# BadgerTechnologies/navigation

Hardware: AMD Instinct MI355X
Metric: scored trajectories/sec (whole node) + costmap inflation cells/sec, 400x400 map (higher is better)
Workload: dtype f64

## Files before the change

### navigation_amd/csrc/planner_score.h

```cpp
#pragma once
#include "planner_common.h"

namespace navgpu {

__host__ __device__ inline size_t score_bits_bytes(int win) {
  return (((size_t)4 * win * ((win + 31) >> 5) * 4) + 15) & ~(size_t)15;
}
__host__ __device__ inline size_t score_scratch_bytes(int win) { return score_bits_bytes(win); }
__device__ __forceinline__ int divSmall(int n, int d) {
  int q = (int)((float)n * __builtin_amdgcn_rcpf((float)d));
  int r = n - q * d;
  if (r < 0) {
    --q;
    r += d;
  }
  if (r >= d) ++q;
  return q;
}

struct WorldToMapFast {
  const Geom& g;
  const double& inv_res;
  __device__ __forceinline__ bool operator()(double wx, double wy, uint32_t& mx, uint32_t& my) const {
    const double dx = wx - g.ox, dy = wy - g.oy;
    const double qx = dx * inv_res, qy = dy * inv_res;
    double fx = floor(qx), fy = floor(qy);
    const double rx = qx - fx, ry = qy - fy;
    if (__builtin_expect(fmin(rx, ry) < 1.0e-7 || fmax(rx, ry) > 1.0 - 1.0e-7, 0)) {
      fx = !(dx >= 0.0) ? -1.0 : (qx >= 1.0e6 ? 1.0e6 : (double)(int)(dx / g.res));
      fy = !(dy >= 0.0) ? -1.0 : (qy >= 1.0e6 ? 1.0e6 : (double)(int)(dy / g.res));
    }
    int ix, iy;
    asm("v_cvt_i32_f64 %0, %1" : "=v"(ix) : "v"(fx));
    asm("v_cvt_i32_f64 %0, %1" : "=v"(iy) : "v"(fy));
    mx = (uint32_t)ix;
    my = (uint32_t)iy;
    return mx < g.nx && my < g.ny;
  }
};

__device__ __forceinline__ void addCritic(double& total, bool en, double value, double scale) {
  if (!en) return;
  double cost = value;
  if (cost != 0) cost *= scale;
  total += cost;
}

constexpr uint32_t kScoreAuxBytes = 64;
__host__ __device__ inline uint32_t score_prep_reject_bytes(const PlannerDev& pl) { return (pl.max_axis * pl.max_axis + 255u) & ~255u; }
__host__ __device__ inline uint32_t score_prep_reject_offset(const PlannerDev& pl) { return pl.prep_stride - score_prep_reject_bytes(pl); }
template <size_t kAllowAbove = 48 * 1024, typename... P, typename... A>
void launchScore(void (*kernel)(P...), dim3 grid, int threads, size_t lds, hipStream_t s, A... args) {
  if (lds > kAllowAbove) hipFuncSetAttribute((const void*)kernel, hipFuncAttributeMaxDynamicSharedMemorySize, (int)lds);
  hipLaunchKernelGGL(kernel, grid, dim3(threads), lds, s, args...);
}
size_t score_table_row_bytes(const PlannerDev& pl);
size_t score_table_lds_bytes(const PlannerDev& pl);
bool score_sweep_applies(const PlannerDev& pl);
uint32_t launch_score_sweep(const PlannerDev& pl, uint32_t first, uint32_t count, hipStream_t s);

}
```

### navigation_amd/csrc/planner_score.hip

```cpp
#include "planner_score.h"

namespace navgpu {

#ifdef NAVGPU_PREP_TIMING
__device__ unsigned long long g_prep_stats[16];
#define PREP_STAMP(i) prep_t[i] = wall_clock64()
#else
#define PREP_STAMP(i)
#endif

struct ScoreRobot {
  uint32_t inst;
  Geom g;
  navgpu_robot_state st;
  const uint8_t* master;
  const uint32_t *dpath, *dgoal, *dfront;
  const int32_t* cnt;
  uint32_t nfp;
  int win, wx0, wy0;
  int win_bytes, nw;
};
__device__ __forceinline__ ScoreRobot scoreRobot(const PlannerDev& pl, uint32_t inst) {
  ScoreRobot r;
  r.inst = inst;
// ... 200 lines not shown
  for (uint32_t i = threadIdx.x; i < n16; i += blockDim.x) img[i] = lds[i];
}

__device__ __forceinline__ void storeSweepScalars(const PlannerDev& pl, const ScoreRobot& r, const float (*s_axis)[kMaxAxis], int* s_cnt,
                                                  const uint8_t* s_dyn) {
  const uint32_t tid = threadIdx.x;
  const navgpu_dwa_config& c = pl.cfg;
  const Geom& g = r.g;
  const int32_t* cnt = r.cnt;
  const uint32_t inst = r.inst;
  const int win = r.win, wx0 = r.wx0, wy0 = r.wy0, nw = r.nw;
  const uint32_t* s_fb = reinterpret_cast<const uint32_t*>(s_dyn + r.win_bytes);
  uint8_t* rej = pl.prep + (size_t)inst * pl.prep_stride + score_prep_reject_offset(pl);
  int32_t* aux = reinterpret_cast<int32_t*>(rej - kScoreAuxBytes);
  const int c0 = win / 2;
  const uint32_t w_c0 = (uint32_t)(c0 * nw + (c0 >> 5));
  const int start_fail = ((s_fb[4 * w_c0 + 2] >> (c0 & 31)) & 1u) ? 4 : (((s_fb[4 * w_c0 + 3] >> (c0 & 31)) & 1u) ? 5 : 0);
  if (tid == 0) s_cnt[0] = (win / 2) * (win / 2);
  __syncthreads();
  {
    int dmin = win * win;
    for (int it = tid; it < win * nw; it += blockDim.x) {
      const int y = it / nw, j = it - y * nw;
      uint32_t m = (c.sum_scores ? s_fb[4 * it] : s_fb[4 * it + 1]) | (start_fail == 4 ? 0u : s_fb[4 * it + 2]) | (start_fail != 0 ? 0u : s_fb[4 * it + 3]);
      const int dy = y > c0 ? y - c0 : c0 - y;
      const int p = c0 - 32 * j;
      const uint32_t right = p <= 0 ? m : (p >= 32 ? 0u : m & (0xFFFFFFFFu << p)), left = m & ~right;
      if (right) dmin = min(dmin, (32 * j + __ffs(right) - 1 - c0) * (32 * j + __ffs(right) - 1 - c0) + dy * dy);
      if (left) dmin = min(dmin, (c0 - (32 * j + 31 - __clz(left))) * (c0 - (32 * j + 31 - __clz(left))) + dy * dy);
    }
    atomicMin(&s_cnt[0], dmin);
  }
  __syncthreads();
  if (tid == 0) {
    const double inv_res = pl.inv_res, fpd = c.forward_point_distance;
    const bool en_fwd = pl.scale_goal != 0 || (pl.align_on[inst] && pl.scale_path != 0);
    const uint32_t fwd_margin = (uint32_t)fmin(ceil(fabs(fpd) * inv_res) + 1.0, 1.0e6);
    const bool fwd_screen = !en_fwd || (2u * fwd_margin < g.nx && 2u * fwd_margin < g.ny);
    const uint32_t fwd_lo = en_fwd ? fwd_margin : 0u, fwd_nx = g.nx - 2u * fwd_lo, fwd_ny = g.ny - 2u * fwd_lo;
    const bool need_margin = !((uint32_t)wx0 - fwd_lo < fwd_nx && (uint32_t)(wx0 + win - 1) - fwd_lo < fwd_nx && (uint32_t)wy0 - fwd_lo < fwd_ny &&
                               (uint32_t)(wy0 + win - 1) - fwd_lo < fwd_ny);
    aux[0] = wx0;
    aux[1] = wy0;
    aux[2] = (int32_t)fwd_lo;
    aux[3] = (int32_t)fwd_nx;
    aux[4] = (int32_t)fwd_ny;
    aux[5] = need_margin ? 1 : 0;
    aux[6] = fwd_screen ? 1 : 0;
    aux[7] = (int)floor(sqrt((double)s_cnt[0]));
    aux[8] = start_fail;
  }
  const int nyv = max(cnt[1], 1), nxyv = cnt[0] * cnt[1];
  for (int i = tid; i < nxyv; i += blockDim.x) {
    const int ix = i / nyv, iy = i - ix * nyv;
    const double vmag = hyp2((double)s_axis[0][ix], (double)s_axis[1][iy]);
    const double eps = 1e-4;
    rej[i] = (uint8_t)(((c.min_trans_vel >= 0 && vmag + eps < c.min_trans_vel) ? 1 : 0) | ((c.max_trans_vel >= 0 && vmag - eps > c.max_trans_vel) ? 2 : 0));
  }
}

struct ScoreInputs {
  static constexpr int kAxisChunks = (3 * kMaxAxis + kScoreThreads - 1) / kScoreThreads;
  double fp;
  float axis[kAxisChunks];
};
__device__ __forceinline__ ScoreInputs loadInputs(const PlannerDev& pl, const ScoreRobot& r) {
  const uint32_t tid = threadIdx.x;
  ScoreInputs in;
  in.fp = pl.fp_spec[(size_t)r.inst * kMaxFootprint * 2 + (tid < 2 * r.nfp ? tid : 0)];
#pragma unroll
  for (int u = 0; u < ScoreInputs::kAxisChunks; ++u) {
    const uint32_t i = min(tid + (uint32_t)u * kScoreThreads, 3u * kMaxAxis - 1), a = i / kMaxAxis, k = i - a * kMaxAxis;
    in.axis[u] = pl.axis_samples[((size_t)r.inst * 3 + a) * pl.max_axis + min(k, pl.max_axis - 1)];
    if (k >= pl.max_axis) in.axis[u] = 0.f;
  }
  return in;
}
__device__ __forceinline__ void loadImage(const PlannerDev& pl, const ScoreRobot& r, const ScoreInputs& in, double* s_fp, float (*s_axis)[kMaxAxis],
                                          uint8_t* s_dyn) {
  const uint32_t tid = threadIdx.x;
  const uint4* img = reinterpret_cast<const uint4*>(pl.prep + (size_t)r.inst * pl.prep_stride);
  uint4* lds = reinterpret_cast<uint4*>(s_dyn);
  const uint32_t n16 = pl.prep_bytes >> 4;
  for (uint32_t i = tid; i < n16; i += blockDim.x) lds[i] = img[i];
  if (tid < 2 * r.nfp) s_fp[tid] = in.fp;
#pragma unroll
  for (int u = 0; u < ScoreInputs::kAxisChunks; ++u) {
    const uint32_t i = tid + (uint32_t)u * kScoreThreads;
    if (i < 3u * kMaxAxis) s_axis[i / kMaxAxis][i % kMaxAxis] = in.axis[u];
  }
// ... 599 lines not shown
```

### navigation_amd/csrc/planner_score_sweep.hip

```cpp
#include "planner_score.h"

namespace navgpu {

constexpr int kSweepThreads = NAVGPU_SCORE_TAB_THREADS;
constexpr int kSweepWaves = 6;
#ifndef NAVGPU_SWEEP_BLOCK_STEPS
#define NAVGPU_SWEEP_BLOCK_STEPS 4
#endif
#ifndef NAVGPU_SWEEP_QUEUE
#define NAVGPU_SWEEP_QUEUE 768
#endif
constexpr int kSweepBlockSteps = NAVGPU_SWEEP_BLOCK_STEPS;
constexpr int kSweepQueue = NAVGPU_SWEEP_QUEUE;
constexpr uint32_t kWalkFailed = 0x80000000u;
#ifdef NAVGPU_SWEEP_COUNTS
__device__ unsigned long long g_sweep_counts[16];
#define SW_COUNT(slot_, n_)                                                                    \
  do {                                                                                           \
    const unsigned long long swc_ = (unsigned long long)(n_);                                    \
    if ((threadIdx.x & 63u) == 0) atomicAdd(&g_sweep_counts[slot_], swc_);                       \
  } while (0)
#else
#define SW_COUNT(slot_, n_)
#endif
#ifdef NAVGPU_SWEEP_TIMING
__device__ unsigned long long g_sweep_stats[16];
#define SW_STAMP(v) const unsigned long long v = __builtin_amdgcn_s_memtime()
#define SW_ACC(i, x) sw_t[i] += (x)
#else
#define SW_STAMP(v)
#define SW_ACC(i, x)
#endif

template <int CHUNK, bool TRIGF>
__global__ __launch_bounds__(kSweepThreads, kSweepWaves) void k_score_sweep(PlannerDev pl, uint32_t first) {
  constexpr int THREADS = kSweepThreads;
  extern __shared__ __align__(16) uint8_t s_dyn[];
  uint8_t* s_win = s_dyn;
  __shared__ double s_rc[THREADS / 64];
  __shared__ int s_ri[THREADS / 64];
  __shared__ int s_cnt[2];
  __shared__ float s_qx[kSweepQueue], s_qy[kSweepQueue];
  __shared__ uint32_t s_qt[kSweepQueue];
  __shared__ uint32_t s_obs[THREADS];
  __shared__ uint32_t s_qn[2];
  __shared__ uint32_t s_more[3];

  const uint32_t inst = first + blockIdx.z;
  const uint32_t tid = threadIdx.x;
#ifdef NAVGPU_SWEEP_TIMING
  unsigned long long sw_t[10] = {0, 0, 0, 0, 0, 0, 0, 0, 0, 0};
#endif
  SW_STAMP(sw0);
  __builtin_amdgcn_s_setprio(3);
  const navgpu_dwa_config& c = pl.cfg;
  const Geom g = geomOf(pl, inst);
  const navgpu_robot_state st = pl.state[inst];
  const uint8_t* master = pl.master + (size_t)inst * pl.cells_padded;
  const uint32_t* dpath = pl.path + (size_t)inst * pl.cells;
  const uint32_t* dgoal = pl.goal + (size_t)inst * pl.cells;
  const uint32_t* dfront = pl.goal_front + (size_t)inst * pl.cells;
  const int32_t* cnt = pl.axis_count + 4 * inst;
  const int n_samples = cnt[3];
  const uint32_t nfp = pl.fp_n[inst];
  const int win = (int)pl.win;

  if (tid == 0) s_cnt[0] = s_cnt[1] = 0;
  if (tid < 2) s_qn[tid] = 0;
  if (tid < 3) s_more[tid] = 0;
  s_obs[tid] = 0;
  const uint8_t* rej_bytes = pl.prep + (size_t)inst * pl.prep_stride + score_prep_reject_offset(pl);
  const int32_t* aux = reinterpret_cast<const int32_t*>(rej_bytes - kScoreAuxBytes);
  const int wx0 = aux[0], wy0 = aux[1];
  const uint32_t fwd_lo = (uint32_t)aux[2], fwd_nx = (uint32_t)aux[3], fwd_ny = (uint32_t)aux[4];
  const bool need_margin = aux[5] != 0, fwd_screen = aux[6] != 0;
  const int free_cells = aux[7];
  const int start_fail = aux[8];
  const uint32_t osc = pl.osc_flags[inst];
  const int32_t align_on = pl.align_on[inst];
  const int win_bytes = (win * win + 15) & ~15;
  const int nw = (win + 31) >> 5;
  const bool walk_swap = pl.cfg.allow_unknown != 0;
  const uint32_t walk_fail = walk_swap ? 255u : 254u;
  const int K = (int)pl.tab_steps;
  const int tnfp = (int)pl.tab_nfp;
  const int lrows = (int)pl.tab_rows;
  double* s_trig = reinterpret_cast<double*>(s_dyn + win_bytes + score_bits_bytes(win));
  double* s_rot = s_trig + (size_t)lrows * K * 4;
  const int nxy = max(cnt[0] * cnt[1], 1);
  const uint32_t part_slot = blockIdx.y * gridDim.x + blockIdx.x;
  const int t_row_base = (int)blockIdx.y * (int)pl.tab_rows;
  const int t_rows = min(max(cnt[2] - t_row_base, 0), (int)pl.tab_rows);
  const int t_li0 = (int)blockIdx.x * THREADS;
  if (t_li0 >= t_rows * nxy) {
    if (tid == 0) {
      pl.part_cost[(size_t)inst * pl.score_blocks + part_slot] = 1.0e300;
      pl.part_index[(size_t)inst * pl.score_blocks + part_slot] = 0x7FFFFFFF;
    }
    return;
  }
  const int li = t_li0 + (int)tid;
  const int t_row = divSmall(li, nxy);
  const int t_r = li - t_row * nxy;
  const int t_ith = t_row_base + t_row;
  const bool in_range = n_samples > 0 && t_row < t_rows;
  const int sidx = t_r * cnt[2] + t_ith;
  const int nyv = max(cnt[1], 1);
  const int s_ix = divSmall(t_r, nyv), s_iy = t_r - s_ix * nyv;
  const float* axis = pl.axis_samples + (size_t)inst * 3 * pl.max_axis;
  const uint32_t amax = pl.max_axis - 1u;
  const float vs0 = axis[min((uint32_t)s_ix, amax)], vs1 = axis[pl.max_axis + min((uint32_t)s_iy, amax)], vs2 = axis[2u * pl.max_axis + min((uint32_t)t_ith, amax)];
  const uint32_t rej_xy = rej_bytes[in_range ? t_r : 0];
  {
    const uint4* img = reinterpret_cast<const uint4*>(pl.prep + (size_t)inst * pl.prep_stride);
    uint4* lds = reinterpret_cast<uint4*>(s_dyn);
    const int last = max(t_rows, 1) - 1;
    const int r0 = min(divSmall(t_li0, nxy), last);
    const int r1 = min(divSmall(t_li0 + THREADS - 1, nxy), last);
    const int n16w = (int)((win_bytes + score_bits_bytes(win)) >> 4);
    const int ncopy = r1 - r0 + 1;
    const int n_trig = ncopy * K * 2, n_rot = ncopy * K * tnfp;
    const int l_trig = n16w + r0 * K * 2, g_trig = n16w + (t_row_base + r0) * K * 2;
    const int l_rot = n16w + lrows * K * 2 + r0 * K * tnfp, g_rot = n16w + (int)pl.tab_nth * K * 2 + (t_row_base + r0) * K * tnfp;
    const int ia0 = (int)tid, ia1 = (int)tid + THREADS;
    const uint4 va0 = img[min(ia0, n16w - 1)], va1 = img[min(ia1, n16w - 1)];
    const uint4 vb = img[g_trig + min((int)tid, n_trig - 1)], vc = img[g_rot + min((int)tid, max(n_rot, 1) - 1)];
    if (ia0 < n16w) lds[ia0] = va0;
    if (ia1 < n16w) lds[ia1] = va1;
    if ((int)tid < n_trig) lds[l_trig + (int)tid] = vb;
    if ((int)tid < n_rot) lds[l_rot + (int)tid] = vc;
    if (n16w > 2 * THREADS || n_trig > THREADS || n_rot > THREADS) {
      for (int i = (int)tid + 2 * THREADS; i < n16w; i += THREADS) lds[i] = img[i];
      for (int i = (int)tid + THREADS; i < n_trig; i += THREADS) lds[l_trig + i] = img[g_trig + i];
      for (int i = (int)tid + THREADS; i < n_rot; i += THREADS) lds[l_rot + i] = img[g_rot + i];
    }
  }
  SW_STAMP(sw1a);
  __syncthreads();
  __builtin_amdgcn_s_setprio(0);
  SW_STAMP(sw1);
  SW_ACC(0, sw1a - sw0);
  SW_ACC(1, sw1 - sw1a);

  auto inWin = [&](int x, int y) { return (unsigned)(x - wx0) < (unsigned)win && (unsigned)(y - wy0) < (unsigned)win; };
  auto cellCost = [&](int x, int y) -> uint8_t {
    const bool in = inWin(x, y);
    uint32_t v = s_win[in ? (y - wy0) * win + (x - wx0) : 0];
    asm volatile("" : "+v"(v));
    if (walk_swap && v >= 254u) v ^= 1u;
    if (__builtin_expect(!in, 0)) v = master[y * g.nx + x];
    return (uint8_t)v;
  };
  const double inv_res = pl.inv_res;
  const WorldToMapFast w2m{g, inv_res};

  auto walkWindow = [&](const double x, const double y, const int te, uint32_t& mx, bool& outside) -> bool {
    const double* rot = s_rot + (size_t)te * tnfp * 2;
    bool off = false;
    outside = false;
    mx = 0;
    uint32_t ux, uy;
    off |= !w2m(x + rot[0], y + rot[1], ux, uy);
    const int fx0 = (int)ux, fy0 = (int)uy;
    int pxc = fx0, pyc = fy0;
    for (uint32_t v = 1; v <= nfp; ++v) {
      int vx = fx0, vy = fy0;
      if (v < nfp) {
        off |= !w2m(x + rot[2 * v], y + rot[2 * v + 1], ux, uy);
        vx = (int)ux;
        vy = (int)uy;
      }
      const int dx = vx - pxc, dy = vy - pyc;
      const int adx = dx < 0 ? -dx : dx, ady = dy < 0 ? -dy : dy;
      const bool xmaj = adx >= ady;
      const int sx = (vx >= pxc) ? 1 : -1, sy = (vy >= pyc) ? win : -win;
      const int den = max(adx, ady), numadd = min(adx, ady), numpixels = den;
      int num = den >> 1;
      const bool in = inWin(pxc, pyc) && inWin(vx, vy);
      outside |= !in;
      const int inc1 = in ? (xmaj ? sy : sx) : 0, inc2 = in ? (xmaj ? sx : sy) : 0;
      int addr = in ? (pyc - wy0) * win + (pxc - wx0) : 0;
      const int addr_first = addr;
      int cp = 0;
      do {
        uint32_t cellv[CHUNK];
#pragma unroll
        for (int u = 0; u < CHUNK; ++u) {
          cellv[u] = s_win[(cp + u <= numpixels) ? addr : addr_first];
          num += numadd;
          const bool ge = num >= den;
          num -= ge ? den : 0;
          addr += (ge ? inc1 : 0) + inc2;
        }
#pragma unroll
        for (int u = 0; u < CHUNK; ++u) mx = max(mx, cellv[u]);
        cp += CHUNK;
      } while (__ballot(cp <= numpixels) != 0ull);
      pxc = vx;
      pyc = vy;
    }
    return off;
  };
  auto walkCostmap = [&](const double x, const double y, const int te) -> uint32_t {
    const double* rot = s_rot + (size_t)te * tnfp * 2;
    uint32_t mx = 0, ux, uy;
    w2m(x + rot[0], y + rot[1], ux, uy);
    const int fx0 = (int)ux, fy0 = (int)uy;
    int pxc = fx0, pyc = fy0;
    for (uint32_t v = 1; v <= nfp; ++v) {
      int vx = fx0, vy = fy0;
      if (v < nfp) {
        w2m(x + rot[2 * v], y + rot[2 * v + 1], ux, uy);
        vx = (int)ux;
        vy = (int)uy;
      }
      int deltax = vx - pxc, deltay = vy - pyc;
      deltax = deltax < 0 ? -deltax : deltax;
      deltay = deltay < 0 ? -deltay : deltay;
      int lx = pxc, ly = pyc;
      int xinc1, xinc2, yinc1, yinc2, den, num, numadd, numpixels;
      xinc1 = xinc2 = (vx >= pxc) ? 1 : -1;
      yinc1 = yinc2 = (vy >= pyc) ? 1 : -1;
      if (deltax >= deltay) {
        xinc1 = 0;
        yinc2 = 0;
        den = deltax;
        num = deltax / 2;
        numadd = deltay;
        numpixels = deltax;
      } else {
        xinc2 = 0;
        yinc1 = 0;
        den = deltay;
        num = deltay / 2;
        numadd = deltax;
        numpixels = deltay;
      }
      for (int cp = 0; cp <= numpixels; ++cp) {
        const uint32_t cc = master[ly * g.nx + lx];
        const uint32_t ct = (walk_swap && cc >= 254u) ? (cc ^ 1u) : cc;
        mx = ct > mx ? ct : mx;
        num += numadd;
        if (num >= den) {
          num -= den;
          lx += xinc1;
          ly += yinc1;
        }
        lx += xinc2;
        ly += yinc2;
      }
      pxc = vx;
      pyc = vy;
    }
    return mx;
  };

  double total = -1.0;
  int status = NAVGPU_SAMPLE_REJECTED;
  const float vs[3] = {vs0, vs1, vs2};
  const bool reject = !in_range || ((rej_xy & 1u) && (c.min_rot_vel >= 0 && fabs((double)vs2) + 1e-4 < c.min_rot_vel)) || (rej_xy & 2u) || K <= 0;
  if (in_range && !reject) status = NAVGPU_SAMPLE_SCORED;
  const double dt = pl.tab_dt;
  const double xv = vs[0], yv = vs[1], thv = vs[2];
  const bool osc_fail = ((osc & NAVGPU_OSC_FORWARD_POS_ONLY) && xv < 0.0) || ((osc & NAVGPU_OSC_FORWARD_NEG_ONLY) && xv > 0.0) ||
                        ((osc & NAVGPU_OSC_STRAFE_POS_ONLY) && yv < 0.0) || ((osc & NAVGPU_OSC_STRAFE_NEG_ONLY) && yv > 0.0) ||
                        ((osc & NAVGPU_OSC_ROT_POS_ONLY) && thv < 0.0) || ((osc & NAVGPU_OSC_ROT_NEG_ONLY) && thv > 0.0);
  const double sc_obs = pl.scale_obstacle, sc_gf = pl.scale_goal, sc_al = align_on ? pl.scale_path : 0.0, sc_path = pl.scale_path,
               sc_goal = pl.scale_goal;
  const bool en_obs = sc_obs != 0, en_gf = sc_gf != 0, en_al = sc_al != 0, en_path = sc_path != 0, en_goal = sc_goal != 0;
  int first_fail = 6;
  int fail_code = 0;
  uint32_t d_gf = 0, d_al = 0, d_path = 0, d_goal = 0;
  uint32_t fail_cell = 0xFFFFFFFFu, last_c = 0, last_f = 0xFFFFFFFFu;
  const double fpd = c.forward_point_distance;
  const uint32_t N_obst = pl.cells, N_unreach = pl.cells + 1;
  if (en_obs && nfp == 0) {
    fail_code = -9;
    first_fail = 1;
  }
  const int min_order = en_obs ? 1 : en_gf ? 2 : en_al ? 3 : en_path ? 4 : en_goal ? 5 : 6;
  uint32_t fb_off = (uint32_t)win_bytes;
  asm volatile("" : "+v"(fb_off));
  const uint4* s_fb4 = reinterpret_cast<const uint4*>(s_dyn + fb_off);
  const bool scr_sum = c.sum_scores != 0;
  const bool screen_on = fwd_screen && (nfp >= 3 || !en_obs);
  float px = st.pos[0], py = st.pos[1];
  int step = 0;
  uint32_t alive_m = (in_range && !reject && !osc_fail && first_fail > min_order) ? 0xFFFFFFFFu : 0u;
#ifdef NAVGPU_SWEEP_X_NOSTEPS
  alive_m = 0;
#endif
  const bool margin_on = __builtin_amdgcn_readfirstlane((int)need_margin) != 0;
  const uint32_t lane = tid & 63u;
  const int te0 = t_row * K;
  const double vxd = vs[0], vyd = vs[1];
  uint32_t scr_z = 0xFFFFFFFFu, scr_w = 0xFFFFFFFFu;
  const uint32_t scr_off = screen_on ? 0u : 0xFFFFFFFFu;
  SW_STAMP(sw2);
  SW_ACC(2, sw2 - sw1);
  int k_free = 0;
  {
    const float spd = sqrtf(vs0 * vs0 + vs1 * vs1) * (float)(dt * inv_res) * 1.0001f + 1.0e-4f;
    int kl = K - 1;
    if (alive_m != 0u) kl = (screen_on && !margin_on && free_cells >= 3) ? (int)fminf((float)(free_cells - 2) / spd, (float)(K - 1)) : 0;
    for (int off = 32; off > 0; off >>= 1) kl = min(kl, __shfl_xor(kl, off));
    k_free = __builtin_amdgcn_readfirstlane(kl);
  }
  for (int k = 0; k < k_free; ++k) {
    const int te = te0 + k;
    const double cs = s_trig[4 * te], sn = s_trig[4 * te + 1], cs2 = s_trig[4 * te + 2], sn2 = s_trig[4 * te + 3];
    const double tx = TRIGF ? (double)(vs[0] * (float)cs) : vxd * cs, ty = TRIGF ? (double)(vs[0] * (float)sn) : vxd * sn;
    const float nxp = (float)(px + (tx + vyd * cs2) * dt);
    const float nyp = (float)(py + (ty + vyd * sn2) * dt);
    px = nxp;
    py = nyp;
  }
  if (alive_m != 0u) step = k_free;
  SW_COUNT(9, k_free);
  SW_COUNT(10, (unsigned)k_free * (unsigned)__popcll(__ballot(alive_m != 0u)));
  if (k_free > 0 && start_fail != 0 && alive_m != 0u) {
    first_fail = start_fail;
    fail_code = 0;
    fail_cell = (uint32_t)(wy0 + win / 2) * g.nx + (uint32_t)(wx0 + win / 2);
    scr_z = first_fail > 4 ? 0xFFFFFFFFu : 0u;
    scr_w = 0u;
    alive_m = first_fail > min_order ? 0xFFFFFFFFu : 0u;
  }
  for (uint32_t blk = 0;; ++blk) {
    SW_STAMP(sb0);
    if (__ballot(alive_m != 0u) != 0ull) {
      for (int it = 0; it < kSweepBlockSteps; ++it) {
        const int sc = min(step, K - 1);
        const int te = te0 + sc;
        const double x = px, y = py;
        const double cs = s_trig[4 * te], sn = s_trig[4 * te + 1];
        SW_COUNT(4, 1);
        SW_COUNT(8, __popcll(__ballot(alive_m != 0u)));
        const double cs2 = s_trig[4 * te + 2], sn2 = s_trig[4 * te + 3];
        const double tx = TRIGF ? (double)(vs[0] * (float)cs) : vxd * cs, ty = TRIGF ? (double)(vs[0] * (float)sn) : vxd * sn;
        const float nxp = (float)(px + (tx + vyd * cs2) * dt);
        const float nyp = (float)(py + (ty + vyd * sn2) * dt);
        uint32_t cx, cy;
        const bool ok_c = w2m(x, y, cx, cy);
        const uint32_t lx = cx - (uint32_t)wx0, ly = cy - (uint32_t)wy0;
        bool in_w = max(lx, ly) < (uint32_t)win;
        uint32_t force = (sc == K - 1) ? 0xFFFFFFFFu : scr_off;
        if (margin_on) {
          in_w = in_w && ok_c;
          if (!((cx - fwd_lo < fwd_nx) && (cy - fwd_lo < fwd_ny))) force = 0xFFFFFFFFu;
        }
        const uint32_t fb_i = in_w ? ly * (uint32_t)nw + (lx >> 5) : 0u;
        const uint4 fbw = s_fb4[fb_i];
        const uint32_t any = (scr_sum ? fbw.x : fbw.y) | (fbw.z & scr_z) | (fbw.w & scr_w) | force | (in_w ? 0u : 0xFFFFFFFFu);
        const bool unscr = ((any >> (lx & 31u)) & alive_m & 1u) != 0u;
        px = nxp;
        py = nyp;
        step -= (int)alive_m;
        if (__ballot(unscr) != 0ull) {
          SW_STAMP(ss0);
          SW_COUNT(3, 1);
          SW_COUNT(0, __popcll(__ballot(unscr)));
          auto sel = [](uint32_t m, uint32_t a, uint32_t b) { return (a & m) | (b & ~m); };
          const uint32_t u = unscr ? 0xFFFFFFFFu : 0u;
          const uint32_t m_last = sc == K - 1 ? 0xFFFFFFFFu : 0u;
          const uint32_t m_on = ok_c ? 0xFFFFFFFFu : 0u;
          const uint32_t m_inw = in_w ? 0xFFFFFFFFu : 0u;
          const uint32_t bit = lx & 31u;
          const uint32_t b_nf = 0u - ((fbw.x >> bit) & 1u), b_cf = 0u - ((fbw.y >> bit) & 1u), b_z = 0u - ((fbw.z >> bit) & 1u), b_w = 0u - ((fbw.w >> bit) & 1u);
          uint32_t m_stall = 0u;
          if (en_obs) {
            const uint32_t m_off = u & ~m_on;
            first_fail = (int)sel(m_off, 1u, (uint32_t)first_fail);
            fail_code = (int)sel(m_off, (uint32_t)-6, (uint32_t)fail_code);
            if (nfp < 3) {
              if ((u & m_on) != 0u) {
                const uint8_t cc = cellCost(cx, cy);
                if (cc == kLethal || cc == kInscribed || (cc == kNoInfo && c.allow_unknown == 0)) {
                  fail_code = -6;
                  first_fail = 1;
                } else if (scr_sum || m_last != 0u) {
                  atomicAdd(&s_obs[tid], (uint32_t)cc);
                }
              }
            } else {
              uint32_t m_need = u & m_on & ((b_nf & ((scr_sum ? 0xFFFFFFFFu : 0u) | m_last | b_cf)) | ~m_inw);
#ifdef NAVGPU_SWEEP_X_NOWALK
              m_need = 0u;
#endif
              const unsigned long long pm = __ballot(m_need != 0u);
#ifdef NAVGPU_SWEEP_COUNTS
              {
                const unsigned long long pc = __ballot(m_need != 0u && (scr_sum || m_last != 0u)), pl_ = __ballot(m_need != 0u && m_last != 0u);
                if (lane == 0) {
                  atomicAdd(&g_sweep_counts[1], (unsigned long long)__popcll(pm & ~pc));
                  atomicAdd(&g_sweep_counts[2], (unsigned long long)__popcll(pc));
                  atomicAdd(&g_sweep_counts[11], (unsigned long long)__popcll(pl_));
                }
              }
#endif
              if (pm != 0ull) {
                const int leader = __ffsll((long long)pm) - 1;
                uint32_t base = 0;
                if ((int)lane == leader) base = atomicAdd(&s_qn[blk & 1u], (uint32_t)__popcll(pm));
                base = (uint32_t)__builtin_amdgcn_readlane((int)base, leader);
                const uint32_t slot = base + (uint32_t)__popcll(pm & ((1ull << lane) - 1ull));
                m_stall = m_need & (slot >= (uint32_t)kSweepQueue ? 0xFFFFFFFFu : 0u);
                if ((m_need & ~m_stall) != 0u) {
                  s_qx[slot] = (float)x;
                  s_qy[slot] = (float)y;
                  s_qt[slot] = tid | ((uint32_t)sc << 10) | ((uint32_t)t_row << 17) | (((scr_sum ? 0xFFFFFFFFu : 0u) | m_last) & 0x80000000u);
                }
#ifdef NAVGPU_SWEEP_COUNTS
                if (m_stall != 0u) atomicAdd(&g_sweep_counts[12], 1ull);
#endif
              }
            }
          }
          const uint32_t m_go = u & ~m_stall & (first_fail > 1 ? 0xFFFFFFFFu : 0u);
          {
            const uint32_t live_p = (en_path && 4 < first_fail) ? 0xFFFFFFFFu : 0u, live_g = (en_goal && 5 < first_fail) ? 0xFFFFFFFFu : 0u;
            const uint32_t m_pg = m_go & (live_p | live_g);
            const uint32_t m_pgoff = m_pg & ~m_on, m_pgon = m_pg & m_on;
            const uint32_t cell = cy * g.nx + cx;
            last_c = sel(m_pgon & m_last, cell, last_c);
            const uint32_t m_scr = m_pgon & ~m_last & m_inw;
            const uint32_t hz = m_scr & live_p & b_z, hw = m_scr & ~hz & live_g & b_w;
            const uint32_t ff_off = sel(live_p, 4u, 5u);
            first_fail = (int)sel(m_pgoff, ff_off, sel(hz, 4u, sel(hw, 5u, (uint32_t)first_fail)));
            fail_code = (int)sel(m_pgoff, (uint32_t)-4, sel(hz | hw, 0u, (uint32_t)fail_code));
            fail_cell = sel(hz | hw, cell, fail_cell);
            const uint32_t m_out = m_pgon & ~m_last & ~m_inw;
            if (__ballot(m_out != 0u) != 0ull) {
              if (m_out != 0u) {
                if (en_path && 4 < first_fail) {
                  const uint32_t d = dpath[cell];
                  if (d == N_obst || d == N_unreach) {
                    fail_code = d == N_obst ? -3 : -2;
                    first_fail = 4;
                  }
                }
                if (en_goal && 5 < first_fail) {
                  const uint32_t d = dgoal[cell];
                  if (d == N_obst || d == N_unreach) {
                    fail_code = d == N_obst ? -3 : -2;
                    first_fail = 5;
                  }
                }
              }
            }
            const uint32_t live_f = ((en_gf && 2 < first_fail) || (en_al && 3 < first_fail)) ? 0xFFFFFFFFu : 0u;
            const uint32_t m_fwd = m_go & live_f & (m_last | (margin_on ? 0xFFFFFFFFu : 0u) | ~m_inw);
            if (__ballot(m_fwd != 0u) != 0ull) {
              if (m_fwd != 0u) {
                double sx = x, sy = y;
                if (fpd != 0.0) {
                  sx = x + fpd * cs;
                  sy = y + fpd * sn;
                }
                uint32_t ux, uy;
                if (!w2m(sx, sy, ux, uy)) {
                  fail_code = -4;
                  first_fail = (en_gf && 2 < first_fail) ? 2 : 3;
                } else if (m_last != 0u) {
                  last_f = uy * g.nx + ux;
                }
              }
            }
            last_f = sel(m_go & ~m_fwd & m_last, 0u, last_f);
          }
          scr_z = first_fail > 4 ? 0xFFFFFFFFu : 0u;
          scr_w = first_fail > 5 ? 0xFFFFFFFFu : 0u;
          px = m_stall != 0u ? (float)x : px;
          py = m_stall != 0u ? (float)y : py;
          step = (int)sel(m_stall, (uint32_t)sc, (uint32_t)step);
          alive_m &= first_fail > min_order ? 0xFFFFFFFFu : 0u;
// ... 32 lines not shown
      const bool off = walkWindow(x, y, te, mx_cost, outside);
      if (__builtin_expect(outside && !off, 0)) mx_cost = walkCostmap(x, y, te);
#ifdef NAVGPU_SWEEP_COUNTS
      atomicAdd(&g_sweep_counts[5], 1ull);
      if (off || mx_cost >= walk_fail) atomicAdd(&g_sweep_counts[6], 1ull);
      if (!(off || mx_cost >= walk_fail) && !(tag >> 31)) atomicAdd(&g_sweep_counts[13], 1ull);
      if ((tid & 63u) == (uint32_t)(__ffsll((long long)__ballot(true)) - 1)) atomicAdd(&g_sweep_counts[7], 1ull);
#endif
      if (off || mx_cost >= walk_fail) {
        atomicOr(&s_obs[owner], kWalkFailed);
      } else if (tag >> 31) {
        const double f_cost = (walk_swap && mx_cost == 254u) ? 255.0 : (double)mx_cost;
        uint32_t cx, cy;
        w2m(x, y, cx, cy);
        const double occ = fmax(fmax(0.0, f_cost), (double)cellCost(cx, cy));
        atomicAdd(&s_obs[owner], (uint32_t)occ);
      }
    }
    SW_STAMP(sb3);
    SW_ACC(6, sb3 - sb2);
    __syncthreads();
    SW_STAMP(sb4);
    SW_ACC(7, sb4 - sb3);
    if ((s_obs[tid] & kWalkFailed) != 0u && first_fail > 1) {
      fail_code = -6;
      first_fail = 1;
      alive_m = 0;
    }
    if (!more) break;
  }

  {
    const bool reached = last_f != 0xFFFFFFFFu && first_fail > 1;
    const uint32_t cmax = pl.cells - 1u;
    const uint32_t v_fail = (first_fail == 4 ? dpath : dgoal)[min(fail_cell, cmax)];
    const uint32_t v_gf = dfront[min(last_f, cmax)], v_al = dpath[min(last_f, cmax)];
    const uint32_t v_path = dpath[min(last_c, cmax)], v_goal = dgoal[min(last_c, cmax)];
    if ((first_fail == 4 || first_fail == 5) && fail_code == 0) fail_code = v_fail == N_obst ? -3 : -2;
    if (reached) {
      if (en_gf && 2 < first_fail) d_gf = v_gf;
      if (en_al && 3 < first_fail) d_al = v_al;
      if (en_path && 4 < first_fail) {
        if (v_path == N_obst || v_path == N_unreach) {
          fail_code = v_path == N_obst ? -3 : -2;
          first_fail = 4;
        } else
          d_path = v_path;
      }
      if (en_goal && 5 < first_fail) {
        if (v_goal == N_obst || v_goal == N_unreach) {
          fail_code = v_goal == N_obst ? -3 : -2;
          first_fail = 5;
        } else
          d_goal = v_goal;
      }
    }
  }
  if (in_range && !reject) {
    if (osc_fail) {
      total = -5.0;
    } else if (first_fail < 6) {
      total = (double)fail_code;
    } else {
      total = 0.0;
      addCritic(total, en_obs, (double)(s_obs[tid] & ~kWalkFailed), sc_obs);
      addCritic(total, en_gf, (double)d_gf, sc_gf);
      addCritic(total, en_al, (double)d_al, sc_al);
      addCritic(total, en_path, (double)d_path, sc_path);
      addCritic(total, en_goal, (double)d_goal, sc_goal);
    }
  }
  if (in_range && pl.sample_cost) {
    pl.sample_cost[(size_t)inst * pl.max_samples + sidx] = total;
    pl.sample_status[(size_t)inst * pl.max_samples + sidx] = status;
  }

  const bool valid = in_range && status == NAVGPU_SAMPLE_SCORED && total >= 0.0;
  double bc = valid ? total : 1.0e300;
  int bi = valid ? sidx : 0x7FFFFFFF;
  for (int off = 32; off > 0; off >>= 1) {
    double oc = __shfl_down(bc, off);
    int oi = __shfl_down(bi, off);
    if (oc < bc || (oc == bc && oi < bi)) {
      bc = oc;
      bi = oi;
    }
  }
  const unsigned long long m_scored = __ballot(in_range && status == NAVGPU_SAMPLE_SCORED);
  const unsigned long long m_valid = __ballot(valid);
  if ((tid & 63) == 0) {
    s_rc[tid >> 6] = bc;
    s_ri[tid >> 6] = bi;
    atomicAdd(&s_cnt[0], __popcll(m_scored));
    atomicAdd(&s_cnt[1], __popcll(m_valid));
  }
  __syncthreads();
  if (tid == 0) {
    for (int w = 1; w < THREADS / 64; ++w)
      if (s_rc[w] < bc || (s_rc[w] == bc && s_ri[w] < bi)) {
        bc = s_rc[w];
        bi = s_ri[w];
      }
    pl.part_cost[(size_t)inst * pl.score_blocks + part_slot] = bc;
    pl.part_index[(size_t)inst * pl.score_blocks + part_slot] = bi;
    if (s_cnt[0]) atomicAdd(&pl.counters[2 * inst], s_cnt[0]);
    if (s_cnt[1]) atomicAdd(&pl.counters[2 * inst + 1], s_cnt[1]);
  }
#ifdef NAVGPU_SWEEP_TIMING
  if ((tid & 63u) == 0 && (blockIdx.x & 3u) == 1 && (blockIdx.z & 3u) == 2) {
    const unsigned long long sw9 = __builtin_amdgcn_s_memtime();
    sw_t[8] = sw9 - sw0;
    for (int i = 0; i < 10; ++i) atomicAdd(&g_sweep_stats[i], sw_t[i]);
    atomicAdd(&g_sweep_stats[10], 1ull);
  }
#endif
}

static_assert(kSweepThreads <= 1024, "10 bits of lane in the walk queue's tags");
static dim3 score_sweep_grid(const PlannerDev& pl, uint32_t count) {
  const uint32_t rows = std::max(pl.tab_rows, 1u);
  const uint32_t max_nxy = pl.max_samples / std::max(pl.tab_nth, 1u), groups = (pl.tab_nth + rows - 1) / rows;
  return dim3((max_nxy * pl.tab_rows + kSweepThreads - 1) / kSweepThreads, groups, count);
}
bool score_sweep_applies(const PlannerDev& pl) {
  const dim3 grid = score_sweep_grid(pl, 1);
  return pl.use_tables && !pl.mg_generic && grid.x * grid.y <= pl.score_blocks;
}
uint32_t launch_score_sweep(const PlannerDev& pl, uint32_t first, uint32_t count, hipStream_t s) {
  const size_t lds = score_window_bytes(pl.win) + score_table_lds_bytes(pl);
  const dim3 grid = score_sweep_grid(pl, count);
  const bool trigf = pl.cfg.rollout_trig != 0;
  if (pl.fp_chunk <= 6)
    launchScore<40 * 1024>(trigf ? k_score_sweep<6, true> : k_score_sweep<6, false>, grid, kSweepThreads, lds, s, pl, first);
  else if (pl.fp_chunk <= 9)
    launchScore<40 * 1024>(trigf ? k_score_sweep<9, true> : k_score_sweep<9, false>, grid, kSweepThreads, lds, s, pl, first);
  else if (pl.fp_chunk <= 12)
    launchScore<40 * 1024>(trigf ? k_score_sweep<12, true> : k_score_sweep<12, false>, grid, kSweepThreads, lds, s, pl, first);
  else
    launchScore<40 * 1024>(trigf ? k_score_sweep<16, true> : k_score_sweep<16, false>, grid, kSweepThreads, lds, s, pl, first);
// ... 26 lines not shown
```

Before: 5.642 billion.

## Precompute per-pair sample flags in prep and slim sweep kernel registers

Result: no change. 5.713 billion (median of 6 runs) (+1.3%).

```diff
diff --git a/navigation_amd/csrc/planner_score.h b/navigation_amd/csrc/planner_score.h
--- a/navigation_amd/csrc/planner_score.h
+++ b/navigation_amd/csrc/planner_score.h
@@ -47,7 +47,12 @@
 }
 
 constexpr uint32_t kScoreAuxBytes = 64;
-__host__ __device__ inline uint32_t score_prep_reject_bytes(const PlannerDev& pl) { return (pl.max_axis * pl.max_axis + 255u) & ~255u; }
+constexpr uint32_t kPairMinTrans = 1u, kPairMaxTrans = 2u, kPairOsc = 4u;
+constexpr uint32_t kRowOsc = 1u, kRowMinRot = 2u;
+constexpr uint32_t kSweepEnObs = 1u, kSweepEnGf = 2u, kSweepEnAl = 4u, kSweepEnPath = 8u, kSweepEnGoal = 16u;
+__host__ __device__ inline uint32_t score_prep_pair_bits_offset(const PlannerDev& pl) { return 8u * pl.max_axis * pl.max_axis; }
+__host__ __device__ inline uint32_t score_prep_row_bits_offset(const PlannerDev& pl) { return 10u * pl.max_axis * pl.max_axis; }
+__host__ __device__ inline uint32_t score_prep_reject_bytes(const PlannerDev& pl) { return (10u * pl.max_axis * pl.max_axis + pl.max_axis + 255u) & ~255u; }
 __host__ __device__ inline uint32_t score_prep_reject_offset(const PlannerDev& pl) { return pl.prep_stride - score_prep_reject_bytes(pl); }
 template <size_t kAllowAbove = 48 * 1024, typename... P, typename... A>
 void launchScore(void (*kernel)(P...), dim3 grid, int threads, size_t lds, hipStream_t s, A... args) {
diff --git a/navigation_amd/csrc/planner_score.hip b/navigation_amd/csrc/planner_score.hip
--- a/navigation_amd/csrc/planner_score.hip
+++ b/navigation_amd/csrc/planner_score.hip
@@ -256,30 +256,62 @@
     atomicMin(&s_cnt[0], dmin);
   }
   __syncthreads();
+  const double inv_res = pl.inv_res, fpd = c.forward_point_distance;
+  const bool align_on = pl.align_on[inst] != 0;
+  const bool en_obs = pl.scale_obstacle != 0, en_gf = pl.scale_goal != 0, en_al = align_on && pl.scale_path != 0, en_path = pl.scale_path != 0,
+             en_goal = pl.scale_goal != 0;
+  const bool en_fwd = en_gf || en_al;
+  const uint32_t fwd_margin = (uint32_t)fmin(ceil(fabs(fpd) * inv_res) + 1.0, 1.0e6);
+  const bool fwd_screen = !en_fwd || (2u * fwd_margin < g.nx && 2u * fwd_margin < g.ny);
+  const uint32_t fwd_lo = en_fwd ? fwd_margin : 0u, fwd_nx = g.nx - 2u * fwd_lo, fwd_ny = g.ny - 2u * fwd_lo;
+  const bool need_margin = !((uint32_t)wx0 - fwd_lo < fwd_nx && (uint32_t)(wx0 + win - 1) - fwd_lo < fwd_nx && (uint32_t)wy0 - fwd_lo < fwd_ny &&
+                             (uint32_t)(wy0 + win - 1) - fwd_lo < fwd_ny);
+  const bool screen_on = fwd_screen && (r.nfp >= 3 || !en_obs);
+  const int free_cells = (int)floor(sqrt((double)s_cnt[0]));
   if (tid == 0) {
-    const double inv_res = pl.inv_res, fpd = c.forward_point_distance;
-    const bool en_fwd = pl.scale_goal != 0 || (pl.align_on[inst] && pl.scale_path != 0);
-    const uint32_t fwd_margin = (uint32_t)fmin(ceil(fabs(fpd) * inv_res) + 1.0, 1.0e6);
-    const bool fwd_screen = !en_fwd || (2u * fwd_margin < g.nx && 2u * fwd_margin < g.ny);
-    const uint32_t fwd_lo = en_fwd ? fwd_margin : 0u, fwd_nx = g.nx - 2u * fwd_lo, fwd_ny = g.ny - 2u * fwd_lo;
-    const bool need_margin = !((uint32_t)wx0 - fwd_lo < fwd_nx && (uint32_t)(wx0 + win - 1) - fwd_lo < fwd_nx && (uint32_t)wy0 - fwd_lo < fwd_ny &&
-                               (uint32_t)(wy0 + win - 1) - fwd_lo < fwd_ny);
+    const uint32_t min_order = en_obs ? 1 : en_gf ? 2 : en_al ? 3 : en_path ? 4 : en_goal ? 5 : 6;
     aux[0] = wx0;
     aux[1] = wy0;
     aux[2] = (int32_t)fwd_lo;
     aux[3] = (int32_t)fwd_nx;
     aux[4] = (int32_t)fwd_ny;
     aux[5] = need_margin ? 1 : 0;
-    aux[6] = fwd_screen ? 1 : 0;
-    aux[7] = (int)floor(sqrt((double)s_cnt[0]));
+    aux[6] = screen_on ? 1 : 0;
+    aux[7] = free_cells;
     aux[8] = start_fail;
-  }
+    aux[9] = (int32_t)((en_obs ? kSweepEnObs : 0u) | (en_gf ? kSweepEnGf : 0u) | (en_al ? kSweepEnAl : 0u) | (en_path ? kSweepEnPath : 0u) |
+                       (en_goal ? kSweepEnGoal : 0u) | (min_order << 8));
+    double* scales = reinterpret_cast<double*>(aux + 10);
+    scales[0] = pl.scale_obstacle;
+    scales[1] = pl.scale_goal;
+    scales[2] = pl.scale_path;
+  }
+  const uint32_t osc = pl.osc_flags[inst];
+  const int K = (int)pl.tab_steps;
+  const float cells_per_step = (float)(pl.tab_dt * inv_res);
+  const bool free_run = screen_on && !need_margin && free_cells >= 3;
+  float2* pair_v = reinterpret_cast<float2*>(rej);
+  uint16_t* pair_bits = reinterpret_cast<uint16_t*>(rej + score_prep_pair_bits_offset(pl));
+  uint8_t* row_bits = rej + score_prep_row_bits_offset(pl);
   const int nyv = max(cnt[1], 1), nxyv = cnt[0] * cnt[1];
   for (int i = tid; i < nxyv; i += blockDim.x) {
     const int ix = i / nyv, iy = i - ix * nyv;
-    const double vmag = hyp2((double)s_axis[0][ix], (double)s_axis[1][iy]);
+    const float vs0 = s_axis[0][ix], vs1 = s_axis[1][iy];
+    const double vmag = hyp2((double)vs0, (double)vs1);
     const double eps = 1e-4;
-    rej[i] = (uint8_t)(((c.min_trans_vel >= 0 && vmag + eps < c.min_trans_vel) ? 1 : 0) | ((c.max_trans_vel >= 0 && vmag - eps > c.max_trans_vel) ? 2 : 0));
+    const bool osc_xy = ((osc & NAVGPU_OSC_FORWARD_POS_ONLY) && vs0 < 0.f) || ((osc & NAVGPU_OSC_FORWARD_NEG_ONLY) && vs0 > 0.f) ||
+                        ((osc & NAVGPU_OSC_STRAFE_POS_ONLY) && vs1 < 0.f) || ((osc & NAVGPU_OSC_STRAFE_NEG_ONLY) && vs1 > 0.f);
+    const float spd = sqrtf(vs0 * vs0 + vs1 * vs1) * cells_per_step * 1.0001f + 1.0e-4f;
+    const uint32_t kl = free_run ? (uint32_t)(int)fminf((float)(free_cells - 2) / spd, (float)(K - 1)) : 0u;
+    const uint32_t bits = ((c.min_trans_vel >= 0 && vmag + eps < c.min_trans_vel) ? kPairMinTrans : 0u) |
+                          ((c.max_trans_vel >= 0 && vmag - eps > c.max_trans_vel) ? kPairMaxTrans : 0u) | (osc_xy ? kPairOsc : 0u);
+    pair_v[i] = make_float2(vs0, vs1);
+    pair_bits[i] = (uint16_t)(bits | ((kl & 0xFFu) << 8));
+  }
+  if ((int)tid < min(cnt[2], (int)pl.max_axis)) {
+    const float vs2 = s_axis[2][tid];
+    const bool osc_th = ((osc & NAVGPU_OSC_ROT_POS_ONLY) && vs2 < 0.f) || ((osc & NAVGPU_OSC_ROT_NEG_ONLY) && vs2 > 0.f);
+    row_bits[tid] = (uint8_t)((osc_th ? kRowOsc : 0u) | ((c.min_rot_vel >= 0 && fabs((double)vs2) + 1e-4 < c.min_rot_vel) ? kRowMinRot : 0u));
   }
 }
 
diff --git a/navigation_amd/csrc/planner_score_sweep.hip b/navigation_amd/csrc/planner_score_sweep.hip
--- a/navigation_amd/csrc/planner_score_sweep.hip
+++ b/navigation_amd/csrc/planner_score_sweep.hip
@@ -32,6 +32,33 @@
 #define SW_ACC(i, x)
 #endif
 
+template <int CTRL>
+__device__ __forceinline__ uint32_t dppMove(uint32_t v) {
+  return (uint32_t)__builtin_amdgcn_update_dpp((int)v, (int)v, CTRL, 0xF, 0xF, false);
+}
+constexpr int kDppRowShr1 = 0x111, kDppRowShr2 = 0x112, kDppRowShr4 = 0x114, kDppRowShr8 = 0x118, kDppRowBcast15 = 0x142, kDppRowBcast31 = 0x143;
+#define NAVGPU_DPP_STAGES(STAGE_) \
+  STAGE_(kDppRowShr1) STAGE_(kDppRowShr2) STAGE_(kDppRowShr4) STAGE_(kDppRowShr8) STAGE_(kDppRowBcast15) STAGE_(kDppRowBcast31)
+__device__ __forceinline__ uint32_t waveMinU32(uint32_t v) {
+#define NAVGPU_STAGE(C_) v = min(v, dppMove<C_>(v));
+  NAVGPU_DPP_STAGES(NAVGPU_STAGE)
+#undef NAVGPU_STAGE
+  return (uint32_t)__builtin_amdgcn_readlane((int)v, 63);
+}
+__device__ __forceinline__ unsigned long long waveMinU64(unsigned long long v) {
+  uint32_t lo = (uint32_t)v, hi = (uint32_t)(v >> 32);
+#define NAVGPU_STAGE(C_)                                                       \
+  {                                                                            \
+    const uint32_t tl = dppMove<C_>(lo), th = dppMove<C_>(hi);                  \
+    const bool lt = (((unsigned long long)th << 32) | tl) < (((unsigned long long)hi << 32) | lo); \
+    lo = lt ? tl : lo;                                                         \
+    hi = lt ? th : hi;                                                         \
+  }
+  NAVGPU_DPP_STAGES(NAVGPU_STAGE)
+#undef NAVGPU_STAGE
+  return ((unsigned long long)(uint32_t)__builtin_amdgcn_readlane((int)hi, 63) << 32) | (uint32_t)__builtin_amdgcn_readlane((int)lo, 63);
+}
+
 template <int CHUNK, bool TRIGF>
 __global__ __launch_bounds__(kSweepThreads, kSweepWaves) void k_score_sweep(PlannerDev pl, uint32_t first) {
   constexpr int THREADS = kSweepThreads;
@@ -39,7 +66,7 @@
   uint8_t* s_win = s_dyn;
   __shared__ double s_rc[THREADS / 64];
   __shared__ int s_ri[THREADS / 64];
-  __shared__ int s_cnt[2];
+  __shared__ int s_cntw[THREADS / 64][2];
   __shared__ float s_qx[kSweepQueue], s_qy[kSweepQueue];
   __shared__ uint32_t s_qt[kSweepQueue];
   __shared__ uint32_t s_obs[THREADS];
@@ -53,19 +80,18 @@
 #endif
   SW_STAMP(sw0);
   __builtin_amdgcn_s_setprio(3);
-  const navgpu_dwa_config& c = pl.cfg;
   const Geom g = geomOf(pl, inst);
   const navgpu_robot_state st = pl.state[inst];
-  const uint8_t* master = pl.master + (size_t)inst * pl.cells_padded;
-  const uint32_t* dpath = pl.path + (size_t)inst * pl.cells;
-  const uint32_t* dgoal = pl.goal + (size_t)inst * pl.cells;
-  const uint32_t* dfront = pl.goal_front + (size_t)inst * pl.cells;
+  auto robotBase = [&](auto* base, uint32_t stride) {
+    uint32_t i = inst;
+    asm volatile("" : "+s"(i));
+    return base + (size_t)i * stride;
+  };
   const int32_t* cnt = pl.axis_count + 4 * inst;
   const int n_samples = cnt[3];
   const uint32_t nfp = pl.fp_n[inst];
   const int win = (int)pl.win;
 
-  if (tid == 0) s_cnt[0] = s_cnt[1] = 0;
   if (tid < 2) s_qn[tid] = 0;
   if (tid < 3) s_more[tid] = 0;
   s_obs[tid] = 0;
@@ -73,11 +99,9 @@
   const int32_t* aux = reinterpret_cast<const int32_t*>(rej_bytes - kScoreAuxBytes);
   const int wx0 = aux[0], wy0 = aux[1];
   const uint32_t fwd_lo = (uint32_t)aux[2], fwd_nx = (uint32_t)aux[3], fwd_ny = (uint32_t)aux[4];
-  const bool need_margin = aux[5] != 0, fwd_screen = aux[6] != 0;
-  const int free_cells = aux[7];
+  const bool need_margin = aux[5] != 0, screen_on = aux[6] != 0;
   const int start_fail = aux[8];
-  const uint32_t osc = pl.osc_flags[inst];
-  const int32_t align_on = pl.align_on[inst];
+  const uint32_t sweep_flags = (uint32_t)aux[9];
   const int win_bytes = (win * win + 15) & ~15;
   const int nw = (win + 31) >> 5;
   const bool walk_swap = pl.cfg.allow_unknown != 0;
@@ -105,12 +129,11 @@
   const int t_ith = t_row_base + t_row;
   const bool in_range = n_samples > 0 && t_row < t_rows;
   const int sidx = t_r * cnt[2] + t_ith;
-  const int nyv = max(cnt[1], 1);
-  const int s_ix = divSmall(t_r, nyv), s_iy = t_r - s_ix * nyv;
-  const float* axis = pl.axis_samples + (size_t)inst * 3 * pl.max_axis;
-  const uint32_t amax = pl.max_axis - 1u;
-  const float vs0 = axis[min((uint32_t)s_ix, amax)], vs1 = axis[pl.max_axis + min((uint32_t)s_iy, amax)], vs2 = axis[2u * pl.max_axis + min((uint32_t)t_ith, amax)];
-  const uint32_t rej_xy = rej_bytes[in_range ? t_r : 0];
+  const int t_pair = in_range ? t_r : 0;
+  const float2 vs01 = reinterpret_cast<const float2*>(rej_bytes)[t_pair];
+  const uint32_t pair_bits = reinterpret_cast<const uint16_t*>(rej_bytes + score_prep_pair_bits_offset(pl))[t_pair];
+  const uint32_t row_bits = rej_bytes[score_prep_row_bits_offset(pl) + min((uint32_t)t_ith, pl.max_axis - 1u)];
+  const float vs0 = vs01.x, vs1 = vs01.y;
   {
     const uint4* img = reinterpret_cast<const uint4*>(pl.prep + (size_t)inst * pl.prep_stride);
     uint4* lds = reinterpret_cast<uint4*>(s_dyn);
@@ -148,7 +171,7 @@
     uint32_t v = s_win[in ? (y - wy0) * win + (x - wx0) : 0];
     asm volatile("" : "+v"(v));
     if (walk_swap && v >= 254u) v ^= 1u;
-    if (__builtin_expect(!in, 0)) v = master[y * g.nx + x];
+    if (__builtin_expect(!in, 0)) v = robotBase(pl.master, pl.cells_padded)[y * g.nx + x];
     return (uint8_t)v;
   };
   const double inv_res = pl.inv_res;
@@ -203,6 +226,7 @@
   };
   auto walkCostmap = [&](const double x, const double y, const int te) -> uint32_t {
     const double* rot = s_rot + (size_t)te * tnfp * 2;
+    const uint8_t* master = robotBase(pl.master, pl.cells_padded);
     uint32_t mx = 0, ux, uy;
     w2m(x + rot[0], y + rot[1], ux, uy);
     const int fx0 = (int)ux, fy0 = (int)uy;
@@ -257,33 +281,28 @@
 
   double total = -1.0;
   int status = NAVGPU_SAMPLE_REJECTED;
-  const float vs[3] = {vs0, vs1, vs2};
-  const bool reject = !in_range || ((rej_xy & 1u) && (c.min_rot_vel >= 0 && fabs((double)vs2) + 1e-4 < c.min_rot_vel)) || (rej_xy & 2u) || K <= 0;
+  const float vs[2] = {vs0, vs1};
+  const bool reject = !in_range || ((pair_bits & kPairMinTrans) && (row_bits & kRowMinRot)) || (pair_bits & kPairMaxTrans) || K <= 0;
   if (in_range && !reject) status = NAVGPU_SAMPLE_SCORED;
   const double dt = pl.tab_dt;
-  const double xv = vs[0], yv = vs[1], thv = vs[2];
-  const bool osc_fail = ((osc & NAVGPU_OSC_FORWARD_POS_ONLY) && xv < 0.0) || ((osc & NAVGPU_OSC_FORWARD_NEG_ONLY) && xv > 0.0) ||
-                        ((osc & NAVGPU_OSC_STRAFE_POS_ONLY) && yv < 0.0) || ((osc & NAVGPU_OSC_STRAFE_NEG_ONLY) && yv > 0.0) ||
-                        ((osc & NAVGPU_OSC_ROT_POS_ONLY) && thv < 0.0) || ((osc & NAVGPU_OSC_ROT_NEG_ONLY) && thv > 0.0);
-  const double sc_obs = pl.scale_obstacle, sc_gf = pl.scale_goal, sc_al = align_on ? pl.scale_path : 0.0, sc_path = pl.scale_path,
-               sc_goal = pl.scale_goal;
-  const bool en_obs = sc_obs != 0, en_gf = sc_gf != 0, en_al = sc_al != 0, en_path = sc_path != 0, en_goal = sc_goal != 0;
+  const bool osc_fail = (pair_bits & kPairOsc) || (row_bits & kRowOsc);
+  const bool en_obs = sweep_flags & kSweepEnObs, en_gf = sweep_flags & kSweepEnGf, en_al = sweep_flags & kSweepEnAl, en_path = sweep_flags & kSweepEnPath,
+             en_goal = sweep_flags & kSweepEnGoal;
   int first_fail = 6;
   int fail_code = 0;
   uint32_t d_gf = 0, d_al = 0, d_path = 0, d_goal = 0;
   uint32_t fail_cell = 0xFFFFFFFFu, last_c = 0, last_f = 0xFFFFFFFFu;
-  const double fpd = c.forward_point_distance;
+  const double fpd = pl.cfg.forward_point_distance;
   const uint32_t N_obst = pl.cells, N_unreach = pl.cells + 1;
   if (en_obs && nfp == 0) {
     fail_code = -9;
     first_fail = 1;
   }
-  const int min_order = en_obs ? 1 : en_gf ? 2 : en_al ? 3 : en_path ? 4 : en_goal ? 5 : 6;
+  const int min_order = (int)((sweep_flags >> 8) & 7u);
   uint32_t fb_off = (uint32_t)win_bytes;
   asm volatile("" : "+v"(fb_off));
   const uint4* s_fb4 = reinterpret_cast<const uint4*>(s_dyn + fb_off);
-  const bool scr_sum = c.sum_scores != 0;
-  const bool screen_on = fwd_screen && (nfp >= 3 || !en_obs);
+  const bool scr_sum = pl.cfg.sum_scores != 0;
   float px = st.pos[0], py = st.pos[1];
   int step = 0;
   uint32_t alive_m = (in_range && !reject && !osc_fail && first_fail > min_order) ? 0xFFFFFFFFu : 0u;
@@ -298,14 +317,7 @@
   const uint32_t scr_off = screen_on ? 0u : 0xFFFFFFFFu;
   SW_STAMP(sw2);
   SW_ACC(2, sw2 - sw1);
-  int k_free = 0;
-  {
-    const float spd = sqrtf(vs0 * vs0 + vs1 * vs1) * (float)(dt * inv_res) * 1.0001f + 1.0e-4f;
-    int kl = K - 1;
-    if (alive_m != 0u) kl = (screen_on && !margin_on && free_cells >= 3) ? (int)fminf((float)(free_cells - 2) / spd, (float)(K - 1)) : 0;
-    for (int off = 32; off > 0; off >>= 1) kl = min(kl, __shfl_xor(kl, off));
-    k_free = __builtin_amdgcn_readfirstlane(kl);
-  }
+  const int k_free = (int)waveMinU32(alive_m != 0u ? pair_bits >> 8 : (uint32_t)max(K - 1, 0));
   for (int k = 0; k < k_free; ++k) {
     const int te = te0 + k;
     const double cs = s_trig[4 * te], sn = s_trig[4 * te + 1], cs2 = s_trig[4 * te + 2], sn2 = s_trig[4 * te + 3];
@@ -361,6 +373,10 @@
           SW_COUNT(3, 1);
           SW_COUNT(0, __popcll(__ballot(unscr)));
           auto sel = [](uint32_t m, uint32_t a, uint32_t b) { return (a & m) | (b & ~m); };
+          uint32_t fl = sweep_flags;
+          asm volatile("" : "+s"(fl));
+          const bool en_obs = fl & kSweepEnObs, en_gf = fl & kSweepEnGf, en_al = fl & kSweepEnAl, en_path = fl & kSweepEnPath, en_goal = fl & kSweepEnGoal;
+          const int min_order = (int)((fl >> 8) & 7u);
           const uint32_t u = unscr ? 0xFFFFFFFFu : 0u;
           const uint32_t m_last = sc == K - 1 ? 0xFFFFFFFFu : 0u;
           const uint32_t m_on = ok_c ? 0xFFFFFFFFu : 0u;
@@ -375,7 +391,7 @@
             if (nfp < 3) {
               if ((u & m_on) != 0u) {
                 const uint8_t cc = cellCost(cx, cy);
-                if (cc == kLethal || cc == kInscribed || (cc == kNoInfo && c.allow_unknown == 0)) {
+                if (cc == kLethal || cc == kInscribed || (cc == kNoInfo && pl.cfg.allow_unknown == 0)) {
                   fail_code = -6;
                   first_fail = 1;
                 } else if (scr_sum || m_last != 0u) {
@@ -433,14 +449,14 @@
             if (__ballot(m_out != 0u) != 0ull) {
               if (m_out != 0u) {
                 if (en_path && 4 < first_fail) {
-                  const uint32_t d = dpath[cell];
+                  const uint32_t d = robotBase(pl.path, pl.cells)[cell];
                   if (d == N_obst || d == N_unreach) {
                     fail_code = d == N_obst ? -3 : -2;
                     first_fail = 4;
                   }
                 }
                 if (en_goal && 5 < first_fail) {
-                  const uint32_t d = dgoal[cell];
+                  const uint32_t d = robotBase(pl.goal, pl.cells)[cell];
                   if (d == N_obst || d == N_unreach) {
                     fail_code = d == N_obst ? -3 : -2;
                     first_fail = 5;
@@ -539,27 +555,31 @@
 
   {
     const bool reached = last_f != 0xFFFFFFFFu && first_fail > 1;
-    const uint32_t cmax = pl.cells - 1u;
-    const uint32_t v_fail = (first_fail == 4 ? dpath : dgoal)[min(fail_cell, cmax)];
-    const uint32_t v_gf = dfront[min(last_f, cmax)], v_al = dpath[min(last_f, cmax)];
-    const uint32_t v_path = dpath[min(last_c, cmax)], v_goal = dgoal[min(last_c, cmax)];
-    if ((first_fail == 4 || first_fail == 5) && fail_code == 0) fail_code = v_fail == N_obst ? -3 : -2;
-    if (reached) {
-      if (en_gf && 2 < first_fail) d_gf = v_gf;
-      if (en_al && 3 < first_fail) d_al = v_al;
-      if (en_path && 4 < first_fail) {
-        if (v_path == N_obst || v_path == N_unreach) {
-          fail_code = v_path == N_obst ? -3 : -2;
-          first_fail = 4;
-        } else
-          d_path = v_path;
-      }
-      if (en_goal && 5 < first_fail) {
-        if (v_goal == N_obst || v_goal == N_unreach) {
-          fail_code = v_goal == N_obst ? -3 : -2;
-          first_fail = 5;
-        } else
-          d_goal = v_goal;
+    const bool by_screen = (first_fail == 4 || first_fail == 5) && fail_code == 0;
+    if (__ballot(reached || by_screen) != 0ull) {
+      const uint32_t cmax = pl.cells - 1u;
+      const uint32_t *dpath = robotBase(pl.path, pl.cells), *dgoal = robotBase(pl.goal, pl.cells), *dfront = robotBase(pl.goal_front, pl.cells);
+      const uint32_t v_fail = (first_fail == 4 ? dpath : dgoal)[min(fail_cell, cmax)];
+      const uint32_t v_gf = dfront[min(last_f, cmax)], v_al = dpath[min(last_f, cmax)];
+      const uint32_t v_path = dpath[min(last_c, cmax)], v_goal = dgoal[min(last_c, cmax)];
+      if (by_screen) fail_code = v_fail == N_obst ? -3 : -2;
+      if (reached) {
+        if (en_gf && 2 < first_fail) d_gf = v_gf;
+        if (en_al && 3 < first_fail) d_al = v_al;
+        if (en_path && 4 < first_fail) {
+          if (v_path == N_obst || v_path == N_unreach) {
+            fail_code = v_path == N_obst ? -3 : -2;
+            first_fail = 4;
+          } else
+            d_path = v_path;
+        }
+        if (en_goal && 5 < first_fail) {
+          if (v_goal == N_obst || v_goal == N_unreach) {
+            fail_code = v_goal == N_obst ? -3 : -2;
+            first_fail = 5;
+          } else
+            d_goal = v_goal;
+        }
       }
     }
   }
@@ -569,10 +589,13 @@
     } else if (first_fail < 6) {
       total = (double)fail_code;
     } else {
+      const double* scales = reinterpret_cast<const double*>(aux + 10);
+      asm volatile("" : "+s"(scales));
+      const double sc_obs = scales[0], sc_goal = scales[1], sc_path = scales[2];
       total = 0.0;
       addCritic(total, en_obs, (double)(s_obs[tid] & ~kWalkFailed), sc_obs);
-      addCritic(total, en_gf, (double)d_gf, sc_gf);
-      addCritic(total, en_al, (double)d_al, sc_al);
+      addCritic(total, en_gf, (double)d_gf, sc_goal);
+      addCritic(total, en_al, (double)d_al, sc_path);
       addCritic(total, en_path, (double)d_path, sc_path);
       addCritic(total, en_goal, (double)d_goal, sc_goal);
     }
@@ -583,35 +606,33 @@
   }
 
   const bool valid = in_range && status == NAVGPU_SAMPLE_SCORED && total >= 0.0;
-  double bc = valid ? total : 1.0e300;
-  int bi = valid ? sidx : 0x7FFFFFFF;
-  for (int off = 32; off > 0; off >>= 1) {
-    double oc = __shfl_down(bc, off);
-    int oi = __shfl_down(bi, off);
-    if (oc < bc || (oc == bc && oi < bi)) {
-      bc = oc;
-      bi = oi;
-    }
-  }
+  const unsigned long long bc_bits = (unsigned long long)__double_as_longlong(valid ? total : 1.0e300);
+  const unsigned long long wave_bits = waveMinU64(bc_bits);
+  const uint32_t wave_bi = waveMinU32((valid && bc_bits == wave_bits) ? (uint32_t)sidx : 0x7FFFFFFFu);
   const unsigned long long m_scored = __ballot(in_range && status == NAVGPU_SAMPLE_SCORED);
   const unsigned long long m_valid = __ballot(valid);
   if ((tid & 63) == 0) {
-    s_rc[tid >> 6] = bc;
-    s_ri[tid >> 6] = bi;
-    atomicAdd(&s_cnt[0], __popcll(m_scored));
-    atomicAdd(&s_cnt[1], __popcll(m_valid));
+    s_rc[tid >> 6] = __longlong_as_double((long long)wave_bits);
+    s_ri[tid >> 6] = (int)wave_bi;
+    s_cntw[tid >> 6][0] = __popcll(m_scored);
+    s_cntw[tid >> 6][1] = __popcll(m_valid);
   }
   __syncthreads();
   if (tid == 0) {
-    for (int w = 1; w < THREADS / 64; ++w)
+    double bc = s_rc[0];
+    int bi = s_ri[0], n_scored = s_cntw[0][0], n_valid = s_cntw[0][1];
+    for (int w = 1; w < THREADS / 64; ++w) {
       if (s_rc[w] < bc || (s_rc[w] == bc && s_ri[w] < bi)) {
         bc = s_rc[w];
         bi = s_ri[w];
       }
+      n_scored += s_cntw[w][0];
+      n_valid += s_cntw[w][1];
+    }
     pl.part_cost[(size_t)inst * pl.score_blocks + part_slot] = bc;
     pl.part_index[(size_t)inst * pl.score_blocks + part_slot] = bi;
-    if (s_cnt[0]) atomicAdd(&pl.counters[2 * inst], s_cnt[0]);
-    if (s_cnt[1]) atomicAdd(&pl.counters[2 * inst + 1], s_cnt[1]);
+    if (n_scored) atomicAdd(&pl.counters[2 * inst], n_scored);
+    if (n_valid) atomicAdd(&pl.counters[2 * inst + 1], n_valid);
   }
 #ifdef NAVGPU_SWEEP_TIMING
   if ((tid & 63u) == 0 && (blockIdx.x & 3u) == 1 && (blockIdx.z & 3u) == 2) {
```
